# drscotthawley/signaltrain

Hardware: AMD Instinct MI355X
Metric: audio-frames/sec (train step) comp_4c 8192-sample windows @ 1/2/4/8 GPUs (higher is better)
Workload: dtype f32; 1 GPU; comp_4c synthetic, 8192-sample windows, batch 256/GPU, fp32 (BASELINE configs[1]); window=8192, frames_per_window=25, global_batch=256, parallelism=dp1

## Files before the change

signaltrain_amd/csrc/st_misc.h:

```cpp
#pragma once
#include "st_common.h"
#include "st_ae.h"

namespace stm {

__device__ __forceinline__ void fold_row(const float* __restrict__ Sr, const float* __restrict__ Si, float* __restrict__ Sfold,
                                         const int N, const int F, const int KP, const int row)
{
    const int half = KP / 2;
    const bool is_im = row >= half;
    const int k = is_im ? row - half : row;
    const float* S = is_im ? Si : Sr;
    const bool valid = k < F;
    const bool paired = valid && k >= 1 && k <= F - 2;
    const float sgn = is_im ? -1.f : 1.f;
    for (int n4 = threadIdx.x; n4 < N / 4; n4 += blockDim.x) {
        float4 v = make_float4(0.f, 0.f, 0.f, 0.f);
        if (valid) {
            v = reinterpret_cast<const float4*>(S + (size_t)k * N)[n4];
            if (paired) {
                const float4 u = reinterpret_cast<const float4*>(S + (size_t)(N - k) * N)[n4];
                v.x += sgn * u.x; v.y += sgn * u.y; v.z += sgn * u.z; v.w += sgn * u.w;
            }
        }
        reinterpret_cast<float4*>(Sfold + (size_t)row * N)[n4] = v;
    }
}
__global__ void __launch_bounds__(256)
fold_kernel(const float* __restrict__ Sr, const float* __restrict__ Si, float* __restrict__ Sfold, int N, int F, int KP)
{
    fold_row(Sr, Si, Sfold, N, F, KP, blockIdx.x);
}

__device__ __forceinline__ void zero_dead_frame(float* __restrict__ a0, float* __restrict__ a1, float* __restrict__ a2, float* __restrict__ a3,
                                                const int T, const int F, const int t_lo, const int Tv, const int blk)
{
    const int nd = T - Tv;
    const int b = blk / nd, j = blk - b * nd;
    const int t = j < t_lo ? j : j + Tv;
    const size_t base = ((size_t)b * T + t) * F;
    for (int f = threadIdx.x; f < F; f += 256) {
        if (a0) a0[base + f] = 0.f;
        if (a1) a1[base + f] = 0.f;
        if (a2) a2[base + f] = 0.f;
        if (a3) a3[base + f] = 0.f;
    }
}
__global__ void __launch_bounds__(256)
zero_dead_frames_kernel(float* __restrict__ a0, float* __restrict__ a1, float* __restrict__ a2, float* __restrict__ a3,
                        int T, int F, int t_lo, int Tv)
{
    zero_dead_frame(a0, a1, a2, a3, T, F, t_lo, Tv, blockIdx.x);
}

__host__ __device__ __forceinline__ int mae_partial_offset(const int n_loss) { return (n_loss + 3) & ~3; }
template <bool MAE = false>
__global__ void __launch_bounds__(256)
ola_loss_kernel(const float* __restrict__ frs, const float* __restrict__ x, const float* __restrict__ y_true,
                float* __restrict__ y_hat, float* __restrict__ dsyn, float* __restrict__ loss_partial,
                int L, int N, int H, int OT, int ysz, float inv_count, int nslab, size_t slab, int dsyn_pad,
                unsigned short* __restrict__ dsyn16 = nullptr, int ht = 0)
{
    __shared__ float red[4];
    const int b = blockIdx.y;
    const int j = blockIdx.x * 256 + threadIdx.x;
    float lc = 0.f;
    [[maybe_unused]] float ma = 0.f;
    if (j < ysz) {
        int t0 = j / H + 1;
        int t1 = (N + j) / H;
        if (t1 > OT - 1) t1 = OT - 1;
        const float* fb = frs + (size_t)b * OT * N;
        float s = 0.f;
        for (int t = t0; t <= t1; ++t) {
            const size_t o = (size_t)t * N + (N + j - H * t);
            float v[6];
#pragma unroll
            for (int z = 0; z < 6; ++z) v[z] = fb[(z < nslab ? z * slab : 0) + o];
#pragma unroll
            for (int z = 0; z < 6; ++z) s += z < nslab ? v[z] : 0.f;
        }
        const float out = x ? 2.0f * (s + 0.5f * x[(size_t)b * L + (L - ysz) + j]) : s;
        if (y_hat) y_hat[(size_t)b * ysz + j] = out;
        if (y_true) {
            const float dlt = y_true[(size_t)b * ysz + j] - out;
            const float a = fabsf(dlt);
            if (MAE) ma = a;
            if (a < 8.0f) { const float u = expm1f(0.5f * a); const float sh = 0.5f * (u + u / (u + 1.0f)); lc = log1pf(2.0f * sh * sh); }
            else lc = a + log1pf(__expf(-2.0f * a)) - 0.69314718056f;
            if (!MAE) {
                const float ds = -2.0f * tanhf(dlt) * inv_count;
                if (dsyn16) dsyn16[(size_t)b * (ysz + 2 * dsyn_pad) + dsyn_pad + j] = st_to_h16(ds, ht);
                else if (dsyn) dsyn[(size_t)b * (ysz + 2 * dsyn_pad) + dsyn_pad + j] = ds;
            }
        }
    }
    if (!MAE && (dsyn || dsyn16) && dsyn_pad > 0) {
        const size_t ro = (size_t)b * (ysz + 2 * dsyn_pad);
        for (int m = blockIdx.x * 256 + threadIdx.x; m < 2 * dsyn_pad; m += gridDim.x * 256) {
            if (dsyn16) dsyn16[ro + (m < dsyn_pad ? m : ysz + m)] = 0;
            else dsyn[ro + (m < dsyn_pad ? m : ysz + m)] = 0.f;
        }
    }
    if (loss_partial) {
        const int lane = threadIdx.x & 63, g = lane & ~3;
        const float a0 = __shfl(lc, g), a1 = __shfl(lc, g + 1), a2 = __shfl(lc, g + 2), a3 = __shfl(lc, g + 3);
        float q = ((a0 + a1) + a2) + a3;
#pragma unroll
        for (int o = 4; o < 64; o <<= 1) q += __shfl_xor(q, o);
        if (lane == 0) red[threadIdx.x >> 6] = q;
        __syncthreads();
        if (threadIdx.x == 0) loss_partial[blockIdx.y * gridDim.x + blockIdx.x] = (red[0] + red[1]) + (red[2] + red[3]);
    }
    if (MAE) {
        __shared__ float redm[4];
        const int lane = threadIdx.x & 63, g = lane & ~3;
        const float a0 = __shfl(ma, g), a1 = __shfl(ma, g + 1), a2 = __shfl(ma, g + 2), a3 = __shfl(ma, g + 3);
        float q = ((a0 + a1) + a2) + a3;
#pragma unroll
        for (int o = 4; o < 64; o <<= 1) q += __shfl_xor(q, o);
        if (lane == 0) redm[threadIdx.x >> 6] = q;
        __syncthreads();
        if (threadIdx.x == 0) loss_partial[mae_partial_offset(gridDim.y * gridDim.x) + blockIdx.y * gridDim.x + blockIdx.x] = (redm[0] + redm[1]) + (redm[2] + redm[3]);
    }
}

template <int NS, bool MAE = false>
__global__ void __launch_bounds__(256)
ola_loss4_kernel(const float* __restrict__ frs, const float* __restrict__ x, const float* __restrict__ y_true,
                 float* __restrict__ y_hat, float* __restrict__ dsyn, float* __restrict__ loss_partial,
                 int L, int N, int H, int OT, int ysz, float inv_count, size_t slab, int dsyn_pad, int nslot,
                 unsigned short* __restrict__ dsyn16 = nullptr, int ht = 0)
{
    const int b = blockIdx.y;
    const int j = 4 * (blockIdx.x * 256 + threadIdx.x);
    float lc = 0.f;
    [[maybe_unused]] float ma = 0.f;
    if (j < ysz) {
        const int t0 = j / H + 1;
        int t1 = (N + j) / H;
        if (t1 > OT - 1) t1 = OT - 1;
        const float* fb = frs + (size_t)b * OT * N;
        float4 v[3][NS];
#pragma unroll
        for (int u = 0; u < 3; ++u) {
            const int t = t0 + u <= t1 ? t0 + u : t1;
            const size_t o = (size_t)t * N + (size_t)(N + j - H * t);
#pragma unroll
            for (int z = 0; z < NS; ++z) v[u][z] = *reinterpret_cast<const float4*>(fb + z * slab + o);
        }
        float4 xv = make_float4(0.f, 0.f, 0.f, 0.f), yt = xv;
        if (x) xv = *reinterpret_cast<const float4*>(x + (size_t)b * L + (L - ysz) + j);
        if (y_true) yt = *reinterpret_cast<const float4*>(y_true + (size_t)b * ysz + j);
        float s[4] = {0.f, 0.f, 0.f, 0.f};
#pragma unroll
        for (int u = 0; u < 3; ++u) {
            const bool live = t0 + u <= t1;
#pragma unroll
            for (int z = 0; z < NS; ++z) {
                s[0] += live ? v[u][z].x : 0.f; s[1] += live ? v[u][z].y : 0.f; s[2] += live ? v[u][z].z : 0.f; s[3] += live ? v[u][z].w : 0.f;
            }
        }
        const float xs[4] = {xv.x, xv.y, xv.z, xv.w}, ys[4] = {yt.x, yt.y, yt.z, yt.w};
        float out[4], ds[4];
#pragma unroll
        for (int q = 0; q < 4; ++q) {
            out[q] = x ? 2.0f * (s[q] + 0.5f * xs[q]) : s[q];
            const float dlt = ys[q] - out[q];
            const float a = fabsf(dlt);
            float l1;
            if (a < 8.0f) { const float u = expm1f(0.5f * a); const float sh = 0.5f * (u + u / (u + 1.0f)); l1 = log1pf(2.0f * sh * sh); }
            else l1 = a + log1pf(__expf(-2.0f * a)) - 0.69314718056f;
            lc += y_true ? l1 : 0.f;
            if (MAE) ma += y_true ? a : 0.f;
            if (!MAE) ds[q] = -2.0f * tanhf(dlt) * inv_count;
        }
        if (y_hat) *reinterpret_cast<float4*>(y_hat + (size_t)b * ysz + j) = make_float4(out[0], out[1], out[2], out[3]);
        if (!MAE && y_true) {
            const size_t o = (size_t)b * (ysz + 2 * dsyn_pad) + dsyn_pad + j;
            if (dsyn16) *reinterpret_cast<uint2*>(dsyn16 + o) = st_to_h16x4(make_float4(ds[0], ds[1], ds[2], ds[3]), ht);
            else if (dsyn) *reinterpret_cast<float4*>(dsyn + o) = make_float4(ds[0], ds[1], ds[2], ds[3]);
        }
    }
    if (!MAE && (dsyn || dsyn16) && dsyn_pad > 0) {
        const size_t ro = (size_t)b * (ysz + 2 * dsyn_pad);
        for (int m = blockIdx.x * 256 + threadIdx.x; m < 2 * dsyn_pad; m += gridDim.x * 256) {
            if (dsyn16) dsyn16[ro + (m < dsyn_pad ? m : ysz + m)] = 0;
            else dsyn[ro + (m < dsyn_pad ? m : ysz + m)] = 0.f;
        }
    }
    if (loss_partial) {
        float q = lc;
#pragma unroll
        for (int o = 1; o < 64; o <<= 1) q += __shfl_xor(q, o);
        const int slot = 4 * blockIdx.x + (threadIdx.x >> 6);
        if ((threadIdx.x & 63) == 0 && slot < nslot) loss_partial[blockIdx.y * nslot + slot] = q;
    }
    if (MAE) {
        float q = ma;
#pragma unroll
        for (int o = 1; o < 64; o <<= 1) q += __shfl_xor(q, o);
        const int slot = 4 * blockIdx.x + (threadIdx.x >> 6);
        if ((threadIdx.x & 63) == 0 && slot < nslot) loss_partial[mae_partial_offset(gridDim.y * nslot) + blockIdx.y * nslot + slot] = q;
    }
}

__device__ __forceinline__ void pad_scale_block(const float* __restrict__ in, float* __restrict__ out, const int Ls, const int pad, const float s,
                                                const int bx, const int nbx, const int b, unsigned short* __restrict__ out16 = nullptr, const int ht = 0)
{
    const int Lp4 = (Ls + 2 * pad) / 4;
    const float4* src = reinterpret_cast<const float4*>(in + (size_t)b * Ls);
    float4* dst = reinterpret_cast<float4*>(out + (size_t)b * (Ls + 2 * pad));
    uint2* dst16 = reinterpret_cast<uint2*>(out16 + (size_t)b * (Ls + 2 * pad));
    for (int i = bx * 256 + threadIdx.x; i < Lp4; i += nbx * 256) {
        const int j = i - pad / 4;
        float4 v = make_float4(0.f, 0.f, 0.f, 0.f);
        if (j >= 0 && j < Ls / 4) { v = src[j]; v.x *= s; v.y *= s; v.z *= s; v.w *= s; }
        if (out16) dst16[i] = st_to_h16x4(v, ht);
        else dst[i] = v;
    }
}
__global__ void __launch_bounds__(256)
pad_scale_kernel(const float* __restrict__ in, float* __restrict__ out, int Ls, int pad, float s)
{
    pad_scale_block(in, out, Ls, pad, s, blockIdx.x, gridDim.x, blockIdx.y);
}

struct PadJobs { const float* src[4]; float* dst[4]; int rows[4], cols[4], pitch[4], blk0[5]; };
__device__ __forceinline__ void pad_rows4_block(const PadJobs& j, const int blk)
{
    int q = 0;
#pragma unroll
    for (int k = 1; k < 4; ++k) q += blk >= j.blk0[k];
    const int i = (blk - j.blk0[q]) * 256 + threadIdx.x;
    if (i >= j.rows[q] * j.pitch[q]) return;
    const int r = i / j.pitch[q], c = i - r * j.pitch[q];
    j.dst[q][i] = c < j.cols[q] ? j.src[q][r * j.cols[q] + c] : 0.f;
}
struct PrepWide {
    float *Vm, *Vp; int FP, B; unsigned R;
    float *H4Km, *H4Kp; const float* knobs; int K;
    PadJobs pj;
    int n_vpad, n_kn, n_pj;
};
struct PrepArgs {
    const float* x; float* xp; int Ls, pad; float scale; int nbx, n_pad;
    const float* Sr; const float* Si; float* Sfold; float* SfoldT; int N, F, KP, n_fold;
    float *re, *im, *mag, *phs; int T, t_lo, Tv;
    int ht; unsigned short *xp16, *Sfold16, *SfoldT16, *W16; const float* Wr; const float* Wi; int n_w16, n_dead;
    PrepWide wd;
    sta::AEImgJob ai;
};
__device__ __forceinline__ void fold_tile(const float* __restrict__ Sr, const float* __restrict__ Si, float* __restrict__ Sfold,
                                          float* __restrict__ SfoldT, const int N, const int F, const int KP, const int tile,
                                          unsigned short* __restrict__ Sfold16 = nullptr, unsigned short* __restrict__ SfoldT16 = nullptr, const int ht = 0)
{
    __shared__ float tl[32][33];
    const int ntn = N / 32, tk = tile / ntn, tn = tile - tk * ntn;
    const int half = KP / 2;
    const int cx = threadIdx.x & 31, ry = threadIdx.x >> 5;
    float a0[4], a1[4];
#pragma unroll
    for (int j = 0; j < 4; ++j) {
        const int row = tk * 32 + ry + 8 * j, n = tn * 32 + cx;
        const bool is_im = row >= half;
        const int k = is_im ? row - half : row;
        const float* S = is_im ? Si : Sr;
        const int kc = k < F ? k : F - 1, km = (k >= 1 && k <= F - 2) ? N - k : N - 1;
        a0[j] = S[(size_t)kc * N + n]; a1[j] = S[(size_t)km * N + n];
    }
#pragma unroll
    for (int j = 0; j < 4; ++j) {
        const int row = tk * 32 + ry + 8 * j, n = tn * 32 + cx;
        const bool is_im = row >= half;
        const int k = is_im ? row - half : row;
        float v = 0.f;
        if (k < F) {
            v = a0[j];
            if (k >= 1 && k <= F - 2) v += is_im ? -a1[j] : a1[j];
        }
        if (Sfold16) Sfold16[(size_t)row * N + n] = st_to_h16(v, ht); else Sfold[(size_t)row * N + n] = v;
        tl[ry + 8 * j][cx] = v;
    }
    __syncthreads();
#pragma unroll
    for (int j = 0; j < 4; ++j) {
        const int n = tn * 32 + ry + 8 * j, row = tk * 32 + cx;
        if (SfoldT16) SfoldT16[(size_t)n * KP + row] = st_to_h16(tl[cx][ry + 8 * j], ht); else SfoldT[(size_t)n * KP + row] = tl[cx][ry + 8 * j];
    }
}
__global__ void __launch_bounds__(256)
prep_kernel(const PrepArgs a)
{
    const int blk = blockIdx.x;
    if (blk < a.n_pad) { const int b = blk / a.nbx; pad_scale_block(a.x, a.xp, a.Ls, a.pad, a.scale, blk - b * a.nbx, a.nbx, b, a.ht ? a.xp16 : nullptr, a.ht); }
    else if (blk < a.n_pad + a.n_fold) fold_tile(a.Sr, a.Si, a.Sfold, a.SfoldT, a.N, a.F, a.KP, blk - a.n_pad, a.ht ? a.Sfold16 : nullptr, a.ht ? a.SfoldT16 : nullptr, a.ht);
    else if (blk < a.n_pad + a.n_fold + a.n_dead) {
        zero_dead_frame(a.re, a.im, a.mag, a.phs, a.T, a.F, a.t_lo, a.Tv, blk - a.n_pad - a.n_fold);
        if (a.wd.n_vpad) {
            const int nd = a.T - a.Tv, j0 = blk - a.n_pad - a.n_fold, b = j0 / nd, j = j0 - b * nd, t = j < a.t_lo ? j : j + a.Tv;
            const size_t o = (size_t)t * a.wd.R + (size_t)b * a.wd.FP;
            for (int f = threadIdx.x; f < a.wd.FP; f += 256) { a.wd.Vm[o + f] = 0.f; a.wd.Vp[o + f] = 0.f; }
        }
    }
    else if (blk < a.n_pad + a.n_fold + a.n_dead + a.wd.n_vpad) {
        const int np = a.wd.FP - a.F;
        const unsigned idx = (unsigned)(blk - a.n_pad - a.n_fold - a.n_dead) * 256u + threadIdx.x;
        if (np > 0 && idx < (unsigned)a.wd.B * (unsigned)a.T * (unsigned)np) {
            const unsigned bt = idx / (unsigned)np, pcol = idx - bt * (unsigned)np, b = bt / (unsigned)a.T, t = bt - b * (unsigned)a.T;
            const size_t o = (size_t)t * a.wd.R + (size_t)b * a.wd.FP + a.F + pcol;
            a.wd.Vm[o] = 0.f; a.wd.Vp[o] = 0.f;
        }
    }
    else if (blk < a.n_pad + a.n_fold + a.n_dead + a.wd.n_vpad + a.wd.n_kn) {
        const unsigned Q = (unsigned)a.wd.FP / 4, idx = (unsigned)(blk - a.n_pad - a.n_fold - a.n_dead - a.wd.n_vpad) * 256u + threadIdx.x;
        if (idx < (unsigned)a.wd.K * (unsigned)a.wd.B * Q) {
            const unsigned kb = idx / Q, j = idx - kb * Q, k = kb / (unsigned)a.wd.B, b = kb - k * (unsigned)a.wd.B;
            const int f0 = 4 * (int)j;
            const float v = a.wd.knobs[b * a.wd.K + k];
            const float4 q = make_float4(f0 < a.F ? v : 0.f, f0 + 1 < a.F ? v : 0.f, f0 + 2 < a.F ? v : 0.f, f0 + 3 < a.F ? v : 0.f);
            const size_t o = (size_t)(16 + k) * a.wd.R + (size_t)b * a.wd.FP;
            reinterpret_cast<float4*>(a.wd.H4Km + o)[j] = q; reinterpret_cast<float4*>(a.wd.H4Kp + o)[j] = q;
        }
    }
    else if (blk < a.n_pad + a.n_fold + a.n_dead + a.wd.n_vpad + a.wd.n_kn + a.wd.n_pj)
        pad_rows4_block(a.wd.pj, blk - a.n_pad - a.n_fold - a.n_dead - a.wd.n_vpad - a.wd.n_kn);
    else if (blk < a.n_pad + a.n_fold + a.n_dead + a.wd.n_vpad + a.wd.n_kn + a.wd.n_pj + a.ai.n_blk)
        sta::ae_img_build(a.ai, (blk - a.n_pad - a.n_fold - a.n_dead - a.wd.n_vpad - a.wd.n_kn - a.wd.n_pj) * 256 + (int)threadIdx.x);
    else {
        const size_t i4 = (size_t)(blk - a.n_pad - a.n_fold - a.n_dead - a.wd.n_vpad - a.wd.n_kn - a.wd.n_pj - a.ai.n_blk) * 256 + threadIdx.x, n4 = a.N / 4;
        if (i4 < (size_t)2 * a.F * n4) {
            const int jrow = (int)(i4 / n4), c = (int)(i4 - (size_t)jrow * n4);
            const float4 v = reinterpret_cast<const float4*>(((jrow & 1) ? a.Wi : a.Wr) + (size_t)(jrow >> 1) * a.N)[c];
            reinterpret_cast<uint2*>(a.W16 + (size_t)jrow * a.N)[c] = st_to_h16x4(v, a.ht);
        }
    }
}

__global__ void __launch_bounds__(256)
scale_kernel(const float* __restrict__ in, float* __restrict__ out, int64_t n, float s)
{
    for (int64_t i = (int64_t)blockIdx.x * 256 + threadIdx.x; i < n; i += (int64_t)gridDim.x * 256) out[i] = s * in[i];
}

__device__ __forceinline__ void polar_bwd_block(const float* __restrict__ re, const float* __restrict__ im, const float* __restrict__ dmag,
                 const float* __restrict__ dphs, const float* __restrict__ g_mag, float* __restrict__ dG, const int F, const int KP,
                 const float sat,
                 const int bx, const int r, unsigned short* __restrict__ dG16 = nullptr, const int ht = 0)
{
    const int half = KP / 2;
    const int c = bx * 256 + threadIdx.x;
    if (c >= half) return;
    float gre = 0.f, gim = 0.f;
    if (c < F) {
        const size_t i = (size_t)r * F + c;
        const float a = re[i], bb = im[i], dm = dmag[i] + (g_mag ? g_mag[i] : 0.f), dp = dphs[i];
        const float mg = sqrtf(a * a + bb * bb);
        const float inv = mg > 0.f ? 1.0f / mg : 0.f;
        const float rp = a + 1e-7f;
        const float den = rp * rp + bb * bb;
        gre = dm * a * inv - dp * bb / den;
        gim = dm * bb * inv + dp * rp / den;
        if (sat > 0.f) { gre = __builtin_amdgcn_fmed3f(gre, -sat, sat); gim = __builtin_amdgcn_fmed3f(gim, -sat, sat); }
    }
    if (dG16) { dG16[(size_t)r * KP + c] = st_to_h16(gre, ht); dG16[(size_t)r * KP + half + c] = st_to_h16(gim, ht); }
    if (dG) { dG[(size_t)r * KP + c] = gre; dG[(size_t)r * KP + half + c] = gim; }
}
constexpr int POLAR_EPT = 4;
__host__ __device__ static inline unsigned polar_magic(int half) { return (unsigned)((0x100000000ull + (unsigned)half - 1) / (unsigned)half); }
__host__ static inline bool polar_flat_ok(long long R, int half)
{
    const unsigned long long M = polar_magic(half), slack = M * (unsigned)half - 0x100000000ull;
    const unsigned long long total = (unsigned long long)R * (unsigned)half;
    return total < 0x7fffffffull && (slack == 0 || total < 0x100000000ull / slack);
}
__device__ __forceinline__ void polar_bwd_flat(const float* __restrict__ re, const float* __restrict__ im, const float* __restrict__ dmag,
                 const float* __restrict__ dphs, const float* __restrict__ g_mag, float* __restrict__ dG, const int F, const int KP, const float sat,
                 const unsigned bx, const unsigned total, const unsigned magic, unsigned short* __restrict__ dG16, const int ht)
{
    const unsigned half = (unsigned)KP / 2;
    unsigned r[POLAR_EPT], c[POLAR_EPT]; bool on[POLAR_EPT], live[POLAR_EPT];
    float a[POLAR_EPT], bb[POLAR_EPT], dm[POLAR_EPT], dp[POLAR_EPT];
#pragma unroll
    for (int u = 0; u < POLAR_EPT; ++u) {
        const unsigned e = (bx * POLAR_EPT + u) * 256 + threadIdx.x;
        on[u] = e < total;
        r[u] = __umulhi(on[u] ? e : 0u, magic); c[u] = (on[u] ? e : 0u) - r[u] * half;
        live[u] = on[u] && c[u] < (unsigned)F;
        const size_t i = live[u] ? (size_t)r[u] * F + c[u] : 0;
        a[u] = re[i]; bb[u] = im[i]; dm[u] = dmag[i] + (g_mag ? g_mag[i] : 0.f); dp[u] = dphs[i];
    }
#pragma unroll
    for (int u = 0; u < POLAR_EPT; ++u) {
        float gre = 0.f, gim = 0.f;
        if (live[u]) {
            const float mg = sqrtf(a[u] * a[u] + bb[u] * bb[u]);
            const float inv = mg > 0.f ? 1.0f / mg : 0.f;
            const float rp = a[u] + 1e-7f;
            const float den = rp * rp + bb[u] * bb[u];
            gre = dm[u] * a[u] * inv - dp[u] * bb[u] / den;
            gim = dm[u] * bb[u] * inv + dp[u] * rp / den;
            if (sat > 0.f) { gre = __builtin_amdgcn_fmed3f(gre, -sat, sat); gim = __builtin_amdgcn_fmed3f(gim, -sat, sat); }
        }
        if (on[u]) {
            const size_t o = (size_t)r[u] * KP + c[u];
            if (dG16) { dG16[o] = st_to_h16(gre, ht); dG16[o + half] = st_to_h16(gim, ht); }
            if (dG) { dG[o] = gre; dG[o + half] = gim; }
        }
    }
}
__global__ void __launch_bounds__(256)
polar_bwd_kernel(const float* __restrict__ re, const float* __restrict__ im, const float* __restrict__ dmag,
                 const float* __restrict__ dphs, const float* __restrict__ g_mag, float* __restrict__ dG, int R, int F, int KP, const float sat,
                 unsigned short* __restrict__ dG16 = nullptr, const int ht = 0)
{
    polar_bwd_block(re, im, dmag, dphs, g_mag, dG, F, KP, sat, blockIdx.x, blockIdx.y, dG16, ht);
}

struct NyqJob {
    const float* part; int P;
    int on;
};
__device__ __forceinline__ void stage_store4(float* __restrict__ stage, const size_t elem, const float4 v, const int bf16)
{
    if (bf16) {
        typedef __bf16 bf16x2_t __attribute__((ext_vector_type(2)));
        typedef float f32x2_t __attribute__((ext_vector_type(2)));
        union { bf16x2_t h; unsigned u; } lo, hi;
        lo.h = __builtin_convertvector((f32x2_t){v.x, v.y}, bf16x2_t); hi.h = __builtin_convertvector((f32x2_t){v.z, v.w}, bf16x2_t);
        *reinterpret_cast<uint2*>(reinterpret_cast<unsigned short*>(stage) + elem) = make_uint2(lo.u, hi.u);
    } else *reinterpret_cast<float4*>(stage + elem) = v;
}
constexpr int NYQ_CW = 256;
__host__ __device__ static inline int nyq_blocks(int N) { return 2 * ((N + NYQ_CW - 1) / NYQ_CW); }
__host__ __device__ static inline int norm_partial_count(int F, int N) { return 2 * F + nyq_blocks(N); }
__device__ __forceinline__ void
nyquist_chunk(const NyqJob& q, float* __restrict__ gRe, float* __restrict__ gIm, float* __restrict__ norm_partial,
              const int N, const int F, const int blk, const int slot, float* __restrict__ stage, const int stage_bf16 = 0)
{
    __shared__ float4 part[4][64];
    __shared__ float red[4];
    const int per = (N + NYQ_CW - 1) / NYQ_CW;
    const bool is_im = blk >= per;
    const int n4 = (is_im ? blk - per : blk) * (NYQ_CW / 4) + (threadIdx.x & 63), grp = threadIdx.x >> 6;
    float4 v = make_float4(0.f, 0.f, 0.f, 0.f);
    if (4 * n4 < N)
        for (int p0 = grp; p0 < q.P; p0 += 32) {
            float4 u[8];
#pragma unroll
            for (int j = 0; j < 8; ++j) { const int p = p0 + 4 * j < q.P ? p0 + 4 * j : grp; u[j] = *reinterpret_cast<const float4*>(q.part + ((size_t)p * 2 + (is_im ? 1 : 0)) * N + 4 * n4); }
#pragma unroll
            for (int j = 0; j < 8; ++j) if (p0 + 4 * j < q.P) { v.x += u[j].x; v.y += u[j].y; v.z += u[j].z; v.w += u[j].w; }
        }
    part[grp][threadIdx.x & 63] = v;
    __syncthreads();
    float na = 0.f;
    if (threadIdx.x < 64 && 4 * n4 < N) {
        const float4 a = part[0][threadIdx.x], b = part[1][threadIdx.x], c = part[2][threadIdx.x], d = part[3][threadIdx.x];
        v = make_float4((a.x + b.x) + (c.x + d.x), (a.y + b.y) + (c.y + d.y), (a.z + b.z) + (c.z + d.z), (a.w + b.w) + (c.w + d.w));
        *reinterpret_cast<float4*>((is_im ? gIm : gRe) + (size_t)(F - 1) * N + 4 * n4) = v;
        if (stage) stage_store4(stage, (size_t)((is_im ? F : 0) + F - 1) * N + 4 * n4, v, stage_bf16);
        na = fabsf(v.x) + fabsf(v.y) + fabsf(v.z) + fabsf(v.w);
    }
    const float tot = block_sum<4>(na, red);
    if (threadIdx.x == 0) norm_partial[slot] = tot;
}
__device__ __forceinline__ void
wgrad_reduce_block(const float* __restrict__ ws, int nz, float* __restrict__ gRe, float* __restrict__ gIm,
                   float* __restrict__ norm_partial, int N, int F, int KP, int mode, const int row, float* __restrict__ stage, const NyqJob& nyq,
                   const int stage_bf16 = 0)
{
    __shared__ float red[4];
    if (row >= 2 * F) {
        if (nyq.on) nyquist_chunk(nyq, gRe, gIm, norm_partial, N, F, row - 2 * F, row, stage, stage_bf16);
        else if (threadIdx.x == 0) norm_partial[row] = 0.f;
        return;
    }
    const bool is_im = row >= F;
    const int k = is_im ? row - F : row;
    if (nyq.on && k == F - 1) { if (threadIdx.x == 0) norm_partial[row] = 0.f; return; }
    const int src = is_im ? KP / 2 + k : k;
    float* g = is_im ? gIm : gRe;
    const bool mirror = mode == 1 && k >= 1 && k <= F - 2;
    const float sgn = is_im ? -1.f : 1.f;
    const size_t slab = (size_t)KP * N;
    float na = 0.f;
    for (int n4 = threadIdx.x; n4 < N / 4; n4 += blockDim.x) {
        float4 v = make_float4(0.f, 0.f, 0.f, 0.f);
        for (int z0 = 0; z0 < nz; z0 += 8) {
            float4 u[8];
#pragma unroll
            for (int j = 0; j < 8; ++j) { const int z = z0 + j < nz ? z0 + j : nz - 1; u[j] = reinterpret_cast<const float4*>(ws + z * slab + (size_t)src * N)[n4]; }
#pragma unroll
            for (int j = 0; j < 8; ++j) if (z0 + j < nz) { v.x += u[j].x; v.y += u[j].y; v.z += u[j].z; v.w += u[j].w; }
        }
        reinterpret_cast<float4*>(g + (size_t)k * N)[n4] = v;
        if (stage) stage_store4(stage, (size_t)row * N + 4 * n4, v, stage_bf16);
        float a = fabsf(v.x) + fabsf(v.y) + fabsf(v.z) + fabsf(v.w);
        if (mirror) {
            reinterpret_cast<float4*>(g + (size_t)(N - k) * N)[n4] = make_float4(sgn * v.x, sgn * v.y, sgn * v.z, sgn * v.w);
            a *= 2.f;
        }
        na += a;
    }
    const float tot = block_sum<4>(na, red);
    if (threadIdx.x == 0) norm_partial[row] = tot;
}
__global__ void __launch_bounds__(256)
wgrad_reduce_kernel(const float* __restrict__ ws, int nz, float* __restrict__ gRe, float* __restrict__ gIm,
                    float* __restrict__ norm_partial, int N, int F, int KP, int mode, int row0, int nrows, float* __restrict__ stage, const NyqJob nyq,
                    const int extra0 = 0, const int stage_bf16 = 0)
{
    const int row = (int)blockIdx.x < nrows ? (int)blockIdx.x + row0 : 2 * F + extra0 + ((int)blockIdx.x - nrows);
    wgrad_reduce_block(ws, nz, gRe, gIm, norm_partial, N, F, KP, mode, row, stage, nyq, stage_bf16);
}
struct WgradPairArgs { const float* ws[2]; int nz[2]; float* gRe[2]; float* gIm[2]; float* norm[2]; NyqJob nyq[2]; int N, F, KP; };
__global__ void __launch_bounds__(256)
wgrad_pair_reduce_kernel(const WgradPairArgs a)
{
    const int n = norm_partial_count(a.F, a.N);
    if ((int)blockIdx.x < n) wgrad_reduce_block(a.ws[0], a.nz[0], a.gRe[0], a.gIm[0], a.norm[0], a.N, a.F, a.KP, 0, (int)blockIdx.x, nullptr, a.nyq[0]);
    else wgrad_reduce_block(a.ws[1], a.nz[1], a.gRe[1], a.gIm[1], a.norm[1], a.N, a.F, a.KP, 1, (int)blockIdx.x - n, nullptr, a.nyq[1]);
}

__global__ void __launch_bounds__(256)
l1_partial_kernel(const float* __restrict__ g, int64_t n, float scale, float* __restrict__ partial)
{
    __shared__ float red[4];
    float a = 0.f;
    const int64_t n4 = n / 4;
    for (int64_t i = (int64_t)blockIdx.x * 256 + threadIdx.x; i < n4; i += (int64_t)gridDim.x * 256) {
        const float4 v = reinterpret_cast<const float4*>(g)[i];
        a += fabsf(v.x * scale) + fabsf(v.y * scale) + fabsf(v.z * scale) + fabsf(v.w * scale);
    }
    const float tot = block_sum<4>(a, red);
    if (threadIdx.x == 0) partial[blockIdx.x] = tot;
}

__global__ void __launch_bounds__(256)
unstage_l1_kernel(const float* __restrict__ stage, float* __restrict__ gRe, float* __restrict__ gIm, const int F, const int N, const float scale,
                  float* __restrict__ partial, const int n_partial, const int stage_bf16 = 0)
{
    __shared__ float red[4];
    const int row = blockIdx.x;
    const bool is_im = row >= F;
    float* dst = (is_im ? gIm : gRe) + (size_t)(is_im ? row - F : row) * N;
    const float* src = stage + (size_t)row * N;
    float a = 0.f;
    for (int i = threadIdx.x; i < N / 4; i += 256) {
        float4 v;
        if (stage_bf16) {
            const uint2 u = *reinterpret_cast<const uint2*>(reinterpret_cast<const unsigned short*>(stage) + (size_t)row * N + 4 * i);
            v = make_float4(__uint_as_float(u.x << 16), __uint_as_float(u.x & 0xffff0000u), __uint_as_float(u.y << 16), __uint_as_float(u.y & 0xffff0000u));
        } else v = reinterpret_cast<const float4*>(src)[i];
        reinterpret_cast<float4*>(dst)[i] = v;
        a += fabsf(v.x * scale) + fabsf(v.y * scale) + fabsf(v.z * scale) + fabsf(v.w * scale);
    }
    const float tot = block_sum<4>(a, red);
    if (threadIdx.x == 0) partial[row] = tot;
    if (row == 2 * F - 1) for (int j = 2 * F + threadIdx.x; j < n_partial; j += 256) partial[j] = 0.f;
}

__device__ __forceinline__ void ae_grad_reduce_block(const float* __restrict__ ws, const int nparts, const int PG,
                                                     float* __restrict__ g_m, float* __restrict__ g_p, const int bx, const int ae,
                                                     float* __restrict__ norm_out = nullptr, const int slot = 0)
{
    __shared__ float red[4][64];
    const int col = threadIdx.x & 63, pl = threadIdx.x >> 6;
    const int i = bx * 64 + col;
    float s = 0.f;
    if (i < PG) {
        const float* base = ws + (size_t)ae * PG + i;
        const size_t stride = (size_t)2 * PG;
        for (int p0 = pl; p0 < nparts; p0 += 32) {
            float v[8];
#pragma unroll
            for (int u = 0; u < 8; ++u) { const int p = p0 + 4 * u; v[u] = p < nparts ? base[(size_t)p * stride] : 0.f; }
#pragma unroll
            for (int u = 0; u < 8; ++u) s += v[u];
        }
    }
    red[pl][col] = s;
    __syncthreads();
    if (pl != 0) return;
    const float r = i < PG ? (red[0][col] + red[1][col]) + (red[2][col] + red[3][col]) : 0.f;
    if (i < PG) (ae ? g_p : g_m)[i] = r;
    if (norm_out) { const float t = wave_sum(fabsf(r)); if (col == 0) norm_out[slot] = t; }
}
__global__ void __launch_bounds__(256)
ae_grad_reduce_kernel(const float* __restrict__ ws, int nparts, int PG, float* __restrict__ g_m, float* __restrict__ g_p)
{
    ae_grad_reduce_block(ws, nparts, PG, g_m, g_p, blockIdx.x, blockIdx.y);
}
struct PostAeArgs {
    const float* ws; int nparts, PG; float* g_m; float* g_p; int n_red_x, n_red;
    const float* re; const float* im; const float* dmag; const float* dphs; const float* g_mag; float* dG; int F, KP, gx; float sat;
    int n_polar; const float* wg; int wg_nz; float* gSr; float* gSi; float* norm_s; int N; NyqJob nyq;
    unsigned short* dG16; int ht;
    unsigned polar_total, polar_magic;
    float* norm_e;
};
__global__ void __launch_bounds__(256)
post_ae_kernel(const PostAeArgs a)
{
    const int blk = blockIdx.x;
    if (blk < a.n_red) { const int ae = blk / a.n_red_x; ae_grad_reduce_block(a.ws, a.nparts, a.PG, a.g_m, a.g_p, blk - ae * a.n_red_x, ae, a.norm_e, blk); }
    else if (blk < a.n_red + a.n_polar && a.polar_total) polar_bwd_flat(a.re, a.im, a.dmag, a.dphs, a.g_mag, a.dG, a.F, a.KP, a.sat, (unsigned)(blk - a.n_red), a.polar_total, a.polar_magic, a.dG16, a.ht);
    else if (blk < a.n_red + a.n_polar) { const int q = blk - a.n_red, r = q / a.gx; polar_bwd_block(a.re, a.im, a.dmag, a.dphs, a.g_mag, a.dG, a.F, a.KP, a.sat, q - r * a.gx, r, a.dG16, a.ht); }
    else wgrad_reduce_block(a.wg, a.wg_nz, a.gSr, a.gSi, a.norm_s, a.N, a.F, a.KP, 1, blk - a.n_red - a.n_polar, nullptr, a.nyq);
}

struct FinArgs {
    const float* loss_partial; int n_loss; const float* reg_partial; int n_reg;
    const float* norm_a; int n_na; const float* norm_s; int n_ns;
    float inv_ycount, reg_scale, norm_scale;
    const float* norm_e; int n_ne;
};
__device__ __forceinline__ float finalize_block(const FinArgs& f, const bool want_loss, float* red, float& lc, float& rg, float& nrm)
{
    auto psum = [](const float* __restrict__ p, const int n) {
        float s0 = 0.f, s1 = 0.f, s2 = 0.f, s3 = 0.f;
        if ((reinterpret_cast<uintptr_t>(p) & 15) == 0) {
            const int n4 = n >> 2;
            const float4* p4 = reinterpret_cast<const float4*>(p);
            int i = threadIdx.x;
            for (; i + 768 < n4; i += 1024) {
                const float4 u0 = p4[i], u1 = p4[i + 256], u2 = p4[i + 512], u3 = p4[i + 768];
                s0 += (u0.x + u0.y) + (u0.z + u0.w); s1 += (u1.x + u1.y) + (u1.z + u1.w);
                s2 += (u2.x + u2.y) + (u2.z + u2.w); s3 += (u3.x + u3.y) + (u3.z + u3.w);
            }
            for (; i < n4; i += 256) { const float4 u = p4[i]; s0 += (u.x + u.y) + (u.z + u.w); }
            for (int j = 4 * n4 + threadIdx.x; j < n; j += 256) s1 += p[j];
        } else for (int j = threadIdx.x; j < n; j += 256) s0 += p[j];
        return (s0 + s1) + (s2 + s3);
    };
    float a = 0.f, b = 0.f, c = 0.f;
    if (want_loss && f.loss_partial) a = psum(f.loss_partial, f.n_loss);
    if (want_loss && f.reg_partial) b = psum(f.reg_partial, f.n_reg);
    if (f.norm_a) c += psum(f.norm_a, f.n_na);
    if (f.norm_s) c += psum(f.norm_s, f.n_ns);
    if (f.norm_e) c += psum(f.norm_e, f.n_ne);
    if (want_loss) { a = block_sum<4>(a, red); b = block_sum<4>(b, red); }
    c = block_sum<4>(c, red);
    __shared__ float bc;
    if (threadIdx.x == 0) bc = c;
    __syncthreads();
    lc = a * f.inv_ycount; rg = b * f.reg_scale; nrm = bc * f.norm_scale;
    const float coef = 1.0f / (nrm + 1e-6f);
    return coef < 1.0f ? coef : 1.0f;
}
__global__ void __launch_bounds__(256)
finalize_kernel(const FinArgs f, float* __restrict__ scalars)
{
    __shared__ float red[4];
    float lc, rg, nrm;
    const float coef = finalize_block(f, true, red, lc, rg, nrm);
    if (threadIdx.x == 0) {
        if (f.loss_partial) { scalars[1] = lc; scalars[2] = rg; scalars[0] = lc + rg; }
        if (f.norm_a || f.norm_s || f.norm_e) { scalars[3] = nrm; scalars[4] = coef; }
    }
}

__global__ void __launch_bounds__(256)
eval_finalize_kernel(const FinArgs f, const double beta, double* __restrict__ acc)
{
    __shared__ float red[4];
    float lc, rg, nrm, ma, t0, t1;
    finalize_block(f, true, red, lc, rg, nrm);
    FinArgs g = f; g.loss_partial = f.loss_partial + mae_partial_offset(f.n_loss); g.reg_partial = nullptr;
    finalize_block(g, true, red, ma, t0, t1);
    if (threadIdx.x == 0) {
#pragma clang fp contract(off)
        const double loss = (double)(lc + rg), mae = (double)ma;
        acc[0] = beta * acc[0] + (1.0 - beta) * loss;
        acc[1] = loss; acc[2] = (double)lc; acc[3] = (double)rg; acc[4] = mae;
        acc[5] += 1.0; acc[6] += loss; acc[7] += mae;
    }
}

#define ST_ADAM1(c)                                                        \
    {                                                                  \
        const float gg = (sc == 1.0f) ? G.c : G.c * sc;                \
        M.c = M.c + w1 * (gg - M.c);                                   \
        V.c = V.c * b2 + (w2 * gg) * gg;                               \
        const float den = sqrtf(V.c) / bc2_sqrt + eps;                 \
        P.c = P.c + (neg_step_size * M.c) / den;                       \
        G.c = gg;                                                      \
    }
template <bool FIN, bool DEV = false>
__global__ void __launch_bounds__(256)
clip_adam_kernel(float* __restrict__ p, float* __restrict__ g, float* __restrict__ m, float* __restrict__ v,
                 int64_t n4_total, int64_t n4_clip, float* __restrict__ scalars, float grad_scale,
                 float neg_step_size, float w1, float b2, float w2, float bc2_sqrt, float eps, const FinArgs fin, const float b1 = 0.f)
{
    if constexpr (DEV) {
        __shared__ float hs[2];
        if (threadIdx.x == 0) {
            const double st = (double)scalars[6];
            hs[0] = (float)(-(double)scalars[7] / (1.0 - pow((double)b1, st)));
            hs[1] = (float)sqrt(1.0 - pow((double)b2, st));
        }
        __syncthreads();
        neg_step_size = hs[0]; bc2_sqrt = hs[1];
    }
    float coef, nrm;
    if constexpr (FIN) {
        __shared__ float red[4];
        float lc, rg;
        coef = finalize_block(fin, blockIdx.x == 0, red, lc, rg, nrm);
        if (blockIdx.x == 0 && threadIdx.x == 0) {
            if (fin.loss_partial) { scalars[1] = lc; scalars[2] = rg; scalars[0] = lc + rg; }
            scalars[3] = nrm; scalars[4] = coef;
        }
    } else {
        coef = scalars[4]; nrm = scalars[3];
    }
    if (!(nrm <= 3.0e38f)) {
        if (blockIdx.x == 0 && threadIdx.x == 0) scalars[5] = scalars[5] + 1.0f;
        return;
    }
    for (int64_t i = (int64_t)blockIdx.x * 256 + threadIdx.x; i < n4_total; i += (int64_t)gridDim.x * 256) {
        const float sc = (i < n4_clip) ? grad_scale * coef : grad_scale;
        float4 G = reinterpret_cast<float4*>(g)[i];
        float4 M = reinterpret_cast<float4*>(m)[i];
        float4 V = reinterpret_cast<float4*>(v)[i];
        if (G.x == 0.f && G.y == 0.f && G.z == 0.f && G.w == 0.f && M.x == 0.f && M.y == 0.f && M.z == 0.f && M.w == 0.f &&
            V.x == 0.f && V.y == 0.f && V.z == 0.f && V.w == 0.f) continue;
        float4 P = reinterpret_cast<float4*>(p)[i];
        ST_ADAM1(x) ST_ADAM1(y) ST_ADAM1(z) ST_ADAM1(w)
        if (sc != 1.0f) reinterpret_cast<float4*>(g)[i] = G;
        reinterpret_cast<float4*>(m)[i] = M;
        reinterpret_cast<float4*>(v)[i] = V;
        reinterpret_cast<float4*>(p)[i] = P;
    }
}

struct AdamRange { int64_t b4, e4; int clipped; float neg_step, bc2_sqrt; };
struct AdamRanges { AdamRange r[4]; int n; };
__global__ void __launch_bounds__(256)
clip_adam_ranges_kernel(float* __restrict__ p, float* __restrict__ g, float* __restrict__ m, float* __restrict__ v, const AdamRanges tab,
                        float* __restrict__ scalars, const float grad_scale, const float w1, const float b2, const float w2, const float eps, const FinArgs fin)
{
    __shared__ float red[4];
    float lc, rg, nrm;
    const float coef = finalize_block(fin, blockIdx.x == 0, red, lc, rg, nrm);
    if (blockIdx.x == 0 && threadIdx.x == 0) {
        if (fin.loss_partial) { scalars[1] = lc; scalars[2] = rg; scalars[0] = lc + rg; }
        scalars[3] = nrm; scalars[4] = coef;
    }
    if (!(nrm <= 3.0e38f)) {
        if (blockIdx.x == 0 && threadIdx.x == 0) scalars[5] = scalars[5] + 1.0f;
        return;
    }
#pragma unroll
    for (int k = 0; k < 4; ++k) {
        if (k >= tab.n) break;
        const float sc = tab.r[k].clipped ? grad_scale * coef : grad_scale;
        const float neg_step_size = tab.r[k].neg_step, bc2_sqrt = tab.r[k].bc2_sqrt;
        const int64_t e4 = tab.r[k].e4;
        for (int64_t i = tab.r[k].b4 + (int64_t)blockIdx.x * 256 + threadIdx.x; i < e4; i += (int64_t)gridDim.x * 256) {
            float4 G = reinterpret_cast<float4*>(g)[i];
            float4 M = reinterpret_cast<float4*>(m)[i];
            float4 V = reinterpret_cast<float4*>(v)[i];
            if (G.x == 0.f && G.y == 0.f && G.z == 0.f && G.w == 0.f && M.x == 0.f && M.y == 0.f && M.z == 0.f && M.w == 0.f &&
                V.x == 0.f && V.y == 0.f && V.z == 0.f && V.w == 0.f) continue;
            float4 P = reinterpret_cast<float4*>(p)[i];
            ST_ADAM1(x) ST_ADAM1(y) ST_ADAM1(z) ST_ADAM1(w)
            if (sc != 1.0f) reinterpret_cast<float4*>(g)[i] = G;
            reinterpret_cast<float4*>(m)[i] = M;
            reinterpret_cast<float4*>(v)[i] = V;
            reinterpret_cast<float4*>(p)[i] = P;
        }
    }
}
#undef ST_ADAM1


__global__ void step_tick_kernel(float* __restrict__ scalars, const float* __restrict__ lr_table, const int n_lr)
{
    if (threadIdx.x != 0 || blockIdx.x != 0) return;
    const float t = scalars[6] + 1.0f;
    int idx = (int)t - 2; idx = idx < 0 ? 0 : (idx >= n_lr ? n_lr - 1 : idx);
    scalars[6] = t; scalars[7] = lr_table[idx];
}

__device__ __forceinline__ float comp_gain_curve(const float xv, const double thresh, const double ratio)
{
    const float th = (float)thresh, ra = (float)ratio;
    float xdb = 20.0f * log10f(fabsf(xv) + 1e-8f);
    xdb = fmaxf(xdb, -96.0f);
    return xdb > th ? (th + (xdb - th) / ra) - xdb : 0.0f;
}
__device__ __forceinline__ float comp_db_to_lin(const float g) { return exp10f(g / 20.0f); }
constexpr int COMP_CH = 8192;
template <typename XP, typename YP>
__device__ __forceinline__ void
compressor_window_body(XP xb, YP yb, const double thresh, const double ratio, const double alphaA, const double alphaR,
                       const int L, const int ysz, float* __restrict__ g, float* __restrict__ carry_p)
{
    if (threadIdx.x == 0) *carry_p = 0.f;
    for (int c0 = 0; c0 < L; c0 += COMP_CH) {
        const int n = L - c0 < COMP_CH ? L - c0 : COMP_CH;
        for (int i = threadIdx.x; i < n; i += 256) g[i] = comp_gain_curve(xb[c0 + i], thresh, ratio);
        __syncthreads();
        if (threadIdx.x == 0) {
            float prev = *carry_p;
            if (c0 == 0) g[0] = 0.f;
            auto step = [&](float gi_f) {
                const double a = gi_f < prev ? alphaA : alphaR;
                const double gi = gi_f;
                prev = (float)__builtin_fma(a, (double)prev - gi, gi);
                return prev;
            };
            int i = 0;
            if (c0 == 0) {
                for (i = 1; i < 8 && i < n; ++i) g[i] = step(g[i]);
            }
            for (; i + 8 <= n; i += 8) {
                float4 u = *reinterpret_cast<const float4*>(g + i), v = *reinterpret_cast<const float4*>(g + i + 4);
                u.x = step(u.x); u.y = step(u.y); u.z = step(u.z); u.w = step(u.w);
                v.x = step(v.x); v.y = step(v.y); v.z = step(v.z); v.w = step(v.w);
                *reinterpret_cast<float4*>(g + i) = u; *reinterpret_cast<float4*>(g + i + 4) = v;
            }
            for (; i < n; ++i) g[i] = step(g[i]);
            *carry_p = prev;
        }
        __syncthreads();
        for (int i = threadIdx.x; i < n; i += 256) {
            const int j = c0 + i - (L - ysz);
            if (j >= 0) yb[j] = comp_db_to_lin(g[i]) * xb[c0 + i];
        }
        __syncthreads();
    }
}
__device__ __forceinline__ void
compressor_window(const float* __restrict__ xb, float* __restrict__ yb, const double thresh, const double ratio, const double alphaA, const double alphaR,
                  const int L, const int ysz, float* __restrict__ g, float* __restrict__ carry_p)
{
    compressor_window_body<const float* __restrict__, float* __restrict__>(xb, yb, thresh, ratio, alphaA, alphaR, L, ysz, g, carry_p);
}
__device__ __forceinline__ void
compressor_window_inplace(float* xyb, const double thresh, const double ratio, const double alphaA, const double alphaR, const int L,
                          float* __restrict__ g, float* __restrict__ carry_p)
{
    compressor_window_body<const float*, float*>(xyb, xyb, thresh, ratio, alphaA, alphaR, L, L, g, carry_p);
}
__global__ void __launch_bounds__(64)
comp_smooth_kernel(float* __restrict__ gc, const float* __restrict__ kw, const float sr, const int B, const int L)
{
    __shared__ float tile[64][65];
    const int lane = threadIdx.x, b0 = blockIdx.x * 64, b = b0 + lane;
    const int bc = b < B ? b : B - 1;
    const double alphaA = exp(-log(9.0) / ((double)sr * (double)kw[4 * bc + 2]));
    const double alphaR = exp(-log(9.0) / ((double)sr * (double)kw[4 * bc + 3]));
    const int q = lane >> 4, c4 = 4 * (lane & 15);
    float prev = 0.f;
    float4 nx[16];
    auto load = [&](const int c0) {
#pragma unroll
        for (int i = 0; i < 16; ++i) {
            const int r = 4 * i + q;
            nx[i] = *reinterpret_cast<const float4*>(gc + (size_t)(b0 + r < B ? b0 + r : B - 1) * L + c0 + c4);
        }
    };
    load(0);
    for (int c0 = 0; c0 < L; c0 += 64) {
#pragma unroll
        for (int i = 0; i < 16; ++i) {
            const int r = 4 * i + q;
            tile[r][c4] = nx[i].x; tile[r][c4 + 1] = nx[i].y; tile[r][c4 + 2] = nx[i].z; tile[r][c4 + 3] = nx[i].w;
        }
        __syncthreads();
        load(c0 + 64 < L ? c0 + 64 : c0);
        float gv[64];
#pragma unroll
        for (int k = 0; k < 64; ++k) gv[k] = tile[lane][k];
#pragma unroll
        for (int k = 0; k < 64; ++k) {
            if (k == 0 && c0 == 0) { gv[0] = 0.f; continue; }
            const float gi_f = gv[k];
            const double a = gi_f < prev ? alphaA : alphaR;
            const double gi = gi_f;
            prev = (float)__builtin_fma(a, (double)prev - gi, gi);
            gv[k] = prev;
        }
#pragma unroll
        for (int k = 0; k < 64; ++k) tile[lane][k] = gv[k];
        __syncthreads();
#pragma unroll
        for (int i = 0; i < 16; ++i) {
            const int r = 4 * i + q;
            if (b0 + r < B) *reinterpret_cast<float4*>(gc + (size_t)(b0 + r) * L + c0 + c4) = make_float4(tile[r][c4], tile[r][c4 + 1], tile[r][c4 + 2], tile[r][c4 + 3]);
        }
        __syncthreads();
    }
}
__global__ void __launch_bounds__(256)
comp_apply_kernel(const float* __restrict__ x, const float* __restrict__ g, const int L, const int ysz, float* __restrict__ y)
{
    const int b = blockIdx.y, j = blockIdx.x * 256 + threadIdx.x;
    if (j >= ysz) return;
    const size_t i = (size_t)b * L + (L - ysz) + j;
    y[(size_t)b * ysz + j] = comp_db_to_lin(g[i]) * x[i];
}
__global__ void __launch_bounds__(256)
comp_apply_inplace_kernel(float* x, const float* __restrict__ g, const int L)
{
    const size_t r = (size_t)blockIdx.y * L;
    for (int n = blockIdx.x * 256 + threadIdx.x; n < L; n += gridDim.x * 256) x[r + n] = comp_db_to_lin(g[r + n]) * x[r + n];
}
__global__ void __launch_bounds__(256)
compressor_4c_kernel(const float* __restrict__ x, const float* __restrict__ knobs_wc, float sr, int L, int ysz, float* __restrict__ y)
{
    __shared__ __attribute__((aligned(16))) float g[COMP_CH];
    __shared__ float carry;
    const int b = blockIdx.x;
    const double thresh = knobs_wc[4 * b + 0], ratio = knobs_wc[4 * b + 1];
    const double alphaA = exp(-log(9.0) / ((double)sr * (double)knobs_wc[4 * b + 2]));
    const double alphaR = exp(-log(9.0) / ((double)sr * (double)knobs_wc[4 * b + 3]));
    compressor_window(x + (size_t)b * L, y + (size_t)b * ysz, thresh, ratio, alphaA, alphaR, L, ysz, g, &carry);
}

constexpr int ENV_R = 8, ENV_CH = 256 * ENV_R;
struct EnvLds {
    double e[ENV_CH];
    float d[ENV_CH + ENV_CH / ENV_R];
    double wa[4], wb[4];
    double carry; float dcarry;
};
__device__ __forceinline__ float env_db(const float xv) { return 20.0f * log10f(fabsf(xv) + 1e-6f); }
struct EnvCoef { double b0, p; };
__device__ __forceinline__ EnvCoef env_coef(const double attackrel, const double sr)
{
    const double k = tan(1.5707963267948966 / (attackrel * sr));
    return EnvCoef{k / (1.0 + k), (1.0 - k) / (1.0 + k)};
}
__device__ __forceinline__ void
env_compressor_window(const float* __restrict__ xb, const float* __restrict__ db, float* __restrict__ yb, const double thresh, const double ratio,
                      const EnvCoef c, const int L, const int ysz, EnvLds* __restrict__ s)
{
    const int t = threadIdx.x, lane = t & 63, w = t >> 6, i0 = t * ENV_R;
    if (t == 0) { s->carry = 0.0; s->dcarry = 0.f; }
    for (int c0 = 0; c0 < L; c0 += ENV_CH) {
        const int n = L - c0 < ENV_CH ? L - c0 : ENV_CH;
        for (int i = t; i < ENV_CH; i += 256) s->d[i + i / ENV_R] = i < n ? (db ? db[c0 + i] : env_db(xb[c0 + i])) : 0.f;
        __syncthreads();
        float dv[ENV_R];
#pragma unroll
        for (int k = 0; k < ENV_R; ++k) dv[k] = s->d[t * (ENV_R + 1) + k];
        const float dm = t == 0 ? s->dcarry : s->d[t * (ENV_R + 1) - 2];
        double A = 1.0, Bv = 0.0;
#pragma unroll
        for (int k = 0; k < ENV_R; ++k) {
            if (i0 + k >= n) break;
            if (c0 + i0 + k == 0) { A = 0.0; Bv = (double)dv[0]; continue; }
            const double u = c.b0 * ((double)dv[k] + (double)(k ? dv[k - 1] : dm));
            A *= c.p; Bv = __builtin_fma(c.p, Bv, u);
        }
#pragma unroll
        for (int o = 1; o < 64; o <<= 1) {
            const double Ao = __shfl_up(A, o), Bo = __shfl_up(Bv, o);
            if (lane >= o) { Bv = __builtin_fma(A, Bo, Bv); A *= Ao; }
        }
        if (lane == 63) { s->wa[w] = A; s->wb[w] = Bv; }
        double Ae = __shfl_up(A, 1), Be = __shfl_up(Bv, 1);
        if (lane == 0) { Ae = 1.0; Be = 0.0; }
        __syncthreads();
        double e = s->carry;
        for (int v = 0; v < w; ++v) e = __builtin_fma(s->wa[v], e, s->wb[v]);
        e = __builtin_fma(Ae, e, Be);
#pragma unroll
        for (int k = 0; k < ENV_R; ++k) {
            if (i0 + k >= n) break;
            if (c0 + i0 + k == 0) e = (double)dv[0];
            else e = __builtin_fma(c.p, e, c.b0 * ((double)dv[k] + (double)(k ? dv[k - 1] : dm)));
            s->e[i0 + k] = e;
        }
        __syncthreads();
        if (t == 255) { s->carry = e; s->dcarry = dv[ENV_R - 1]; }
        if (c0 + n > L - ysz) {
            for (int i = t; i < n; i += 256) {
                const int j = c0 + i - (L - ysz);
                if (j < 0) continue;
                const double ev = s->e[i];
                const double g = ev > thresh ? exp10((thresh + (ev - thresh) / ratio - ev) / 20.0) : 1.0;
                yb[j] = (float)((double)xb[c0 + i] * g);
            }
        }
    }
}
__global__ void __launch_bounds__(256)
compressor_env_kernel(const float* __restrict__ x, const float* __restrict__ db, const float* __restrict__ knobs_wc, const int kstride, const float sr,
                      const int L, const int ysz, float* __restrict__ y)
{
    __shared__ EnvLds s;
    const int b = blockIdx.x;
    const float* kw = knobs_wc + (size_t)kstride * b;
    env_compressor_window(x + (size_t)b * L, db ? db + (size_t)b * L : nullptr, y + (size_t)b * ysz, (double)kw[0], (double)kw[1],
                          env_coef((double)kw[2], (double)sr), L, ysz, &s);
}


struct AeActsArgs { const float* v; const float* knobs; const float* ae; int w_off[9], b_off[9]; float* out[10]; int B, T, OT, F, K, sf; };
__global__ void __launch_bounds__(64)
ae_acts_kernel(const AeActsArgs a)
{
    const int row = blockIdx.x * 64 + threadIdx.x;
    if (row >= a.B * a.F) return;
    const int b = row / a.F, f = row - b * a.F;
    float h[64 + 16], z[64 + 16];
    const sta::AEShape sh{a.T, a.OT, a.K};
    int outw[9];
    for (int l = 0; l < 9; ++l) outw[l] = sh.out(l);
    int inw = a.T;
    for (int l = 0; l < 9; ++l) {
        const float* W = a.ae + a.w_off[l]; const float* bias = a.ae + a.b_off[l];
        if (l == 4) {
            for (int k = 0; k < a.K; ++k) h[16 + k] = a.knobs[b * a.K + k];
            for (int j = 0; j < 16 + a.K; ++j) a.out[4][(size_t)row * (16 + a.K) + j] = h[j];
            inw = 16 + a.K;
        }
        for (int o = 0; o < outw[l]; ++o) {
            float s = bias[o];
            for (int i = 0; i < inw; ++i) s = __builtin_fmaf(W[o * inw + i], l == 0 ? a.v[((size_t)b * a.T + i) * a.F + f] : h[i], s);
            float e = s > 0.f ? s : expm1f(s);
            if (l == 8) {
                if (a.sf) e *= a.v[((size_t)b * a.T + (a.T - a.OT + o)) * a.F + f];
                a.out[9][(size_t)row * a.OT + o] = e;
            } else z[o] = e;
        }
        if (l == 8) break;
        const int slot = l < 4 ? l : l + 1;
        for (int o = 0; o < outw[l]; ++o) { h[o] = z[o]; a.out[slot][(size_t)row * outw[l] + o] = z[o]; }
        inw = outw[l];
    }
}

__global__ void __launch_bounds__(256)
ola_crop_kernel(const float* __restrict__ frs, float* __restrict__ out, int T, int KW, int hop, int crop, int len)
{
    const int b = blockIdx.y, j = blockIdx.x * 256 + threadIdx.x;
    if (j >= len) return;
    const int p = j + crop;
    int t1 = p / hop; if (t1 > T - 1) t1 = T - 1;
    int t0 = p - KW + 1 <= 0 ? 0 : (p - KW + hop) / hop;
    float s = 0.f;
    for (int t = t0; t <= t1; ++t) s += frs[((size_t)b * T + t) * KW + (p - hop * t)];
    out[(size_t)b * len + j] = s;
}

__global__ void sum_slabs_flat_kernel(const float* __restrict__ ws, int nslab, size_t n, float* __restrict__ out)
{
    const size_t i = (size_t)blockIdx.x * blockDim.x + threadIdx.x;
    if (i >= n) return;
    float s = 0.f;
    for (int z = 0; z < nslab; ++z) s += ws[(size_t)z * n + i];
    out[i] = s;
}

__global__ void col_sum_kernel(const float* __restrict__ X, int R, int C, float* __restrict__ out)
{
    const int c = blockIdx.x * blockDim.x + threadIdx.x;
    if (c >= C) return;
    float s = 0.f;
    for (int r = 0; r < R; ++r) s += X[(size_t)r * C + c];
    out[c] = s;
}

}
```

Measured before the change: 11.45 million frames/s.

## Prefetch Adam operands across finalize, fuse FMAs, reorder wgrad pair block rows

The clip_adam kernel now loads its first G/M/V/P quad before the finalize/grad-norm reduction and software-pipelines later iterations by loading the next quad before computing the current one. The goal is to hide global memory latency behind the reduction and the arithmetic. The Adam moment updates use explicit fmaf, which changes rounding slightly. The wgrad pair reduce kernel also remaps block indices so the Nyquist/extra rows are scheduled first within each half. This costs extra registers, and P is now loaded even for all-zero entries that get skipped.

```diff
diff --git a/signaltrain_amd/csrc/st_misc.h b/signaltrain_amd/csrc/st_misc.h
--- a/signaltrain_amd/csrc/st_misc.h
+++ b/signaltrain_amd/csrc/st_misc.h
@@ -518,9 +518,11 @@
 __global__ void __launch_bounds__(256)
 wgrad_pair_reduce_kernel(const WgradPairArgs a)
 {
-    const int n = norm_partial_count(a.F, a.N);
-    if ((int)blockIdx.x < n) wgrad_reduce_block(a.ws[0], a.nz[0], a.gRe[0], a.gIm[0], a.norm[0], a.N, a.F, a.KP, 0, (int)blockIdx.x, nullptr, a.nyq[0]);
-    else wgrad_reduce_block(a.ws[1], a.nz[1], a.gRe[1], a.gIm[1], a.norm[1], a.N, a.F, a.KP, 1, (int)blockIdx.x - n, nullptr, a.nyq[1]);
+    const int n = norm_partial_count(a.F, a.N), nq = nyq_blocks(a.N);
+    const int half = (int)blockIdx.x >= n, b = (int)blockIdx.x - half * n;
+    const int row = b < nq ? 2 * a.F + b : b - nq;
+    if (!half) wgrad_reduce_block(a.ws[0], a.nz[0], a.gRe[0], a.gIm[0], a.norm[0], a.N, a.F, a.KP, 0, row, nullptr, a.nyq[0]);
+    else wgrad_reduce_block(a.ws[1], a.nz[1], a.gRe[1], a.gIm[1], a.norm[1], a.N, a.F, a.KP, 1, row, nullptr, a.nyq[1]);
 }
 
 __global__ void __launch_bounds__(256)
@@ -681,18 +683,30 @@
 #define ST_ADAM1(c)                                                        \
     {                                                                  \
         const float gg = (sc == 1.0f) ? G.c : G.c * sc;                \
-        M.c = M.c + w1 * (gg - M.c);                                   \
-        V.c = V.c * b2 + (w2 * gg) * gg;                               \
+        M.c = __builtin_fmaf(w1, gg - M.c, M.c);                       \
+        V.c = __builtin_fmaf(gg, w2 * gg, V.c * b2);                   \
         const float den = sqrtf(V.c) / bc2_sqrt + eps;                 \
         P.c = P.c + (neg_step_size * M.c) / den;                       \
         G.c = gg;                                                      \
     }
+struct AdamQuad { float4 G, M, V, P; };
+__device__ __forceinline__ AdamQuad adam_quad_load(const float* p, const float* g, const float* m, const float* v, const int64_t i)
+{
+    AdamQuad q;
+    q.G = reinterpret_cast<const float4*>(g)[i]; q.M = reinterpret_cast<const float4*>(m)[i];
+    q.V = reinterpret_cast<const float4*>(v)[i]; q.P = reinterpret_cast<const float4*>(p)[i];
+    return q;
+}
 template <bool FIN, bool DEV = false>
 __global__ void __launch_bounds__(256)
 clip_adam_kernel(float* __restrict__ p, float* __restrict__ g, float* __restrict__ m, float* __restrict__ v,
                  int64_t n4_total, int64_t n4_clip, float* __restrict__ scalars, float grad_scale,
                  float neg_step_size, float w1, float b2, float w2, float bc2_sqrt, float eps, const FinArgs fin, const float b1 = 0.f)
 {
+    const int64_t stride = (int64_t)gridDim.x * 256;
+    int64_t i = (int64_t)blockIdx.x * 256 + threadIdx.x;
+    AdamQuad nx = {};
+    if (i < n4_total) nx = adam_quad_load(p, g, m, v, i);
     if constexpr (DEV) {
         __shared__ float hs[2];
         if (threadIdx.x == 0) {
@@ -719,19 +733,19 @@
         if (blockIdx.x == 0 && threadIdx.x == 0) scalars[5] = scalars[5] + 1.0f;
         return;
     }
-    for (int64_t i = (int64_t)blockIdx.x * 256 + threadIdx.x; i < n4_total; i += (int64_t)gridDim.x * 256) {
-        const float sc = (i < n4_clip) ? grad_scale * coef : grad_scale;
-        float4 G = reinterpret_cast<float4*>(g)[i];
-        float4 M = reinterpret_cast<float4*>(m)[i];
-        float4 V = reinterpret_cast<float4*>(v)[i];
+    while (i < n4_total) {
+        float4 G = nx.G, M = nx.M, V = nx.V, P = nx.P;
+        const int64_t cur = i;
+        i += stride;
+        if (i < n4_total) nx = adam_quad_load(p, g, m, v, i);
+        const float sc = (cur < n4_clip) ? grad_scale * coef : grad_scale;
         if (G.x == 0.f && G.y == 0.f && G.z == 0.f && G.w == 0.f && M.x == 0.f && M.y == 0.f && M.z == 0.f && M.w == 0.f &&
             V.x == 0.f && V.y == 0.f && V.z == 0.f && V.w == 0.f) continue;
-        float4 P = reinterpret_cast<float4*>(p)[i];
         ST_ADAM1(x) ST_ADAM1(y) ST_ADAM1(z) ST_ADAM1(w)
-        if (sc != 1.0f) reinterpret_cast<float4*>(g)[i] = G;
-        reinterpret_cast<float4*>(m)[i] = M;
-        reinterpret_cast<float4*>(v)[i] = V;
-        reinterpret_cast<float4*>(p)[i] = P;
+        if (sc != 1.0f) reinterpret_cast<float4*>(g)[cur] = G;
+        reinterpret_cast<float4*>(m)[cur] = M;
+        reinterpret_cast<float4*>(v)[cur] = V;
+        reinterpret_cast<float4*>(p)[cur] = P;
     }
 }
 
```

Result: no change. 11.44 million frames/s (-0.2%).
